# Rick0514/SimpleSLAM

Hardware: AMD Instinct MI355X
Metric: scans/s (65 k-pt scan vs 1 M-pt submap, LOAM 10 iters) + pose RMSE vs CPU ref (higher is better)
Workload: dtype f64; 1 GPU; pcr=loam, 65536-pt 64-beam scan vs 1000000-pt submap, 10 GN iters, early exit off, index rebuilt per call (previous call's bounding box and tile layout reused as checked hints), inputs in HBM; parallelism=single GPU, scans_cycled=8

## Files before the change

### simpleslam_amd/csrc/loam.hip

```cpp
#include <hip/hip_ext.h>

#include "pcr_internal.h"
#include "peer_exchange.h"
#include "small_math.h"

namespace pcr {



static constexpr int kNb = 8;
static constexpr uint32_t kNoPos = 0xffffffffu;
static constexpr uint32_t kKeyEmpty = 0xffffffffu;

struct Nb8 {
    double d[kNb];
    uint32_t idx[kNb];
    float x[kNb], y[kNb], z[kNb];
};

__device__ __forceinline__ bool knn_less(double d, uint32_t i, double d2, uint32_t i2) {
    return (d < d2) | ((d == d2) & (i < i2));
}

__device__ __forceinline__ double sqdist(double qx, double qy, double qz, float px, float py, float pz) {
// ... 121 lines not shown
            for (int t = 0; t < 9; ++t) {
                const uint2 r = sh.run[t][tid];
                const uint32_t len = r.y - r.x;
                const bool skip = (uint32_t)t == k && (uint32_t)t < n_runs && rem >= len;
                rem -= skip ? len : 0u; k += skip ? 1u : 0u;
            }
        }
        const uint2 r0 = sh.run[min(k, 9u)][tid];
        cur.k = k; cur.j = r0.x + rem; cur.e = r0.y; cur.nx = sh.run[min(k + 1u, 9u)][tid];
    }
    uint32_t nmax = n_mine;
#pragma unroll
    for (int m = 32; m >= 1; m >>= 1) nmax = max(nmax, (uint32_t)__shfl_xor((int)nmax, m, 64));
    const uint32_t groups = __builtin_amdgcn_readfirstlane((nmax + (uint32_t)kGroup - 1u) / (uint32_t)kGroup);
    float4 c[kGroup];
    if (groups) {
#pragma unroll
        for (int u = 0; u < kGroup; ++u) {
            const uint32_t pos = knn_cursor_step(cur, sh, tid);
            c[u] = pts[(uint32_t)u < n_mine ? pos : 0u];
        }
    }
    if (tl) { float t_ = 0.f; if (groups) { for (int u = 0; u < kGroup; ++u) t_ += c[u].x; } if (t_ == 1.2345e38f) key[0] = 0u; tl[9] = wall_clock64(); }
    for (uint32_t g = 0; g < groups; ++g) {
        float4 n[kGroup];
        if (g + 1u < groups) {
#pragma unroll
            for (int u = 0; u < kGroup; ++u) {
                const uint32_t pos = knn_cursor_step(cur, sh, tid);
                n[u] = pts[(g + 1u) * (uint32_t)kGroup + (uint32_t)u < n_mine ? pos : 0u];
            }
        } else {
#pragma unroll
            for (int u = 0; u < kGroup; ++u) n[u] = make_float4(0.f, 0.f, 0.f, 0.f);
        }
#pragma unroll
        for (int u = 0; u < kGroup; ++u) {
            const uint32_t seq = g * (uint32_t)kGroup + (uint32_t)u;
            const float dx = qxf - c[u].x, dy = qyf - c[u].y, dz = qzf - c[u].z;
            float d = dx * dx;
            d = __builtin_fmaf(dy, dy, d);
            d = __builtin_fmaf(dz, dz, d);
            uint32_t t = (__float_as_uint(d) & ~idmask) | (s0 + seq);
            t = (seq < n_mine && d <= gate_f) ? t : kKeyEmpty;
#pragma unroll
            for (int k = 0; k < kNb; ++k) { const uint32_t lo = min(key[k], t), hi = max(key[k], t); key[k] = lo; t = hi; }
            key[kNb] = min(key[kNb], t);
        }
#pragma unroll
        for (int u = 0; u < kGroup; ++u) c[u] = n[u];
    }
    if (tl) tl[10] = wall_clock64();
    return !inside ? 0 : (too_many ? 2 : 1);
}

__device__ __forceinline__ void knn_decode(const KnnRuns& sh, int tid, const uint32_t key[kNb + 1], uint32_t idmask, uint32_t pos[kNb]) {
    uint32_t P[9], off[9];
    uint32_t acc = 0;
#pragma unroll
    for (int t = 0; t < 9; ++t) { const uint2 r = sh.run[t][tid]; P[t] = acc; off[t] = r.x - acc; acc += r.y - r.x; }
#pragma unroll
    for (int j = 0; j < kNb; ++j) {
        const uint32_t seq = key[j] & idmask;
        uint32_t o = off[0];
#pragma unroll
        for (int t = 1; t < 9; ++t) o = seq >= P[t] ? off[t] : o;
        pos[j] = key[j] == kKeyEmpty ? kNoPos : seq + o;
    }
}

__device__ __forceinline__ double knn_list_bound(const uint32_t key[kNb + 1], uint32_t idmask) {
    if (key[kNb] == kKeyEmpty) return __longlong_as_double(0x7ff0000000000000ll);
    return (double)__uint_as_float(key[kNb] & ~idmask) * (1.0 - 1e-6);
}

struct NnCacheEntry {
    float4 nb[kNb];
    float q0[3];
    float l9;
    double x[3];
    uint32_t pidx[5];
    uint32_t flags;
};
static_assert(sizeof(NnCacheEntry) == 192, "cache entry layout");
static constexpr int kEntryVec = sizeof(NnCacheEntry) / 16;

__device__ __forceinline__ bool knn_from_cache(const NnCacheEntry& ce, double qx, double qy, double qz, Nb8& s, bool* moved) {
#pragma unroll
    for (int j = 0; j < kNb; ++j) {
        const float4 p = ce.nb[j];
        s.x[j] = p.x; s.y[j] = p.y; s.z[j] = p.z; s.idx[j] = __float_as_uint(p.w);
        const double d = sqdist(qx, qy, qz, p.x, p.y, p.z);
        s.d[j] = d == d ? d : __longlong_as_double(0x7ff0000000000000ll);
    }
    bool ord = true;
#pragma unroll
    for (int j = 0; j < 4; ++j) ord = ord & !knn_less(s.d[j + 1], s.idx[j + 1], s.d[j], s.idx[j]);
#pragma unroll
    for (int j = 5; j < kNb; ++j) ord = ord & !knn_less(s.d[j], s.idx[j], s.d[4], s.idx[4]);
    *moved = false;
    if (!__all(ord)) {
        uint32_t before[kNb];
#pragma unroll
        for (int j = 0; j < kNb; ++j) before[j] = s.idx[j];
        nb8_sort(s);
        bool mv = false;
#pragma unroll
        for (int j = 0; j < kNb; ++j) mv = mv | (before[j] != s.idx[j]);
        *moved = mv;
    }
    const double ex = qx - (double)ce.q0[0], ey = qy - (double)ce.q0[1], ez = qz - (double)ce.q0[2];
    const double delta = sqrt(ex * ex + ey * ey + ez * ez) * (1.0 + 1e-12) + 1e-13;
    const double slack = (double)ce.l9 - delta;
    return s.idx[4] != 0xffffffffu && slack > 0.0 && s.d[4] < slack * slack * (1.0 - 1e-12);
}

__device__ __forceinline__ void swap_d(double& a, double& b) { const double t = a; a = b; b = t; }

__device__ __forceinline__ void plane_qr_solve(double a[5][3], double x[3]) {
    double c[5] = {-1.0, -1.0, -1.0, -1.0, -1.0};
    int perm[3] = {0, 1, 2};
    double tau[3] = {0, 0, 0};
    double nu[3], nd[3];
    double maxn = 0;
#pragma unroll
    for (int j = 0; j < 3; ++j) {
        double s = 0;
#pragma unroll
        for (int i = 0; i < 5; ++i) s += a[i][j] * a[i][j];
        nd[j] = nu[j] = sqrt(s);
        if (nu[j] > maxn) maxn = nu[j];
    }
    const double eps = 2.220446049250313e-16;
    const double thr_helper = (maxn * eps) * (maxn * eps) / 5.0;
    const double downdate_thr = 1.4901161193847656e-08;
    int nonzero = 3;
#pragma unroll
    for (int k = 0; k < 3; ++k) {
        int big = k; double bign = nu[k];
#pragma unroll
        for (int j = k + 1; j < 3; ++j) if (nu[j] > bign) { bign = nu[j]; big = j; }
        const double big_sq = bign * bign;
        if (nonzero == 3 && big_sq < thr_helper * (double)(5 - k)) nonzero = k;
#pragma unroll
        for (int j = k + 1; j < 3; ++j) {
            if (big == j) {
#pragma unroll
                for (int i = 0; i < 5; ++i) swap_d(a[i][k], a[i][j]);
                swap_d(nu[k], nu[j]); swap_d(nd[k], nd[j]);
                const int t = perm[k]; perm[k] = perm[j]; perm[j] = t;
            }
        }
        double tail_sq = 0;
#pragma unroll
        for (int i = k + 1; i < 5; ++i) tail_sq += a[i][k] * a[i][k];
        const double c0 = a[k][k];
        const bool tiny = tail_sq <= 2.2250738585072014e-308;
        double beta_h = sqrt(c0 * c0 + tail_sq);
        beta_h = c0 >= 0 ? -beta_h : beta_h;
        const double den = c0 - beta_h;
#pragma unroll
        for (int i = k + 1; i < 5; ++i) { const double q = a[i][k] / den; a[i][k] = tiny ? 0.0 : q; }
        const double tau_h = (beta_h - c0) / beta_h;
        tau[k] = tiny ? 0.0 : tau_h;
        a[k][k] = tiny ? c0 : beta_h;
#pragma unroll
        for (int j = k + 1; j < 3; ++j) {
            double tmp = 0;
// ... 99 lines not shown
            in = d <= seed_sq;
            if (!in) out_min = fmin(out_min, d);
        }
        const unsigned long long m = __ballot(in);
        if (in) tab[n_in + (uint32_t)__popcll(m & ((1ull << lane) - 1ull))] = w;
        n_in += (uint32_t)__popcll(m);
    }
#pragma unroll
    for (int sft = 32; sft >= 1; sft >>= 1) out_min = fmin(out_min, __shfl_xor(out_min, sft, 64));
    __builtin_amdgcn_fence(__ATOMIC_RELEASE, "workgroup");
    for (uint32_t c = lane; c < n_in; c += 64) {
        const WaveCand me = tab[c];
        uint32_t rank = 0;
#pragma unroll 4
        for (uint32_t j = 0; j < n_in; ++j) {
            const WaveCand o = tab[j];
            rank += knn_less(o.d, o.idx, me.d, me.idx) ? 1u : 0u;
        }
        if (rank <= (uint32_t)kNb) { tab[kWaveTab + rank] = me; }
    }
    __builtin_amdgcn_fence(__ATOMIC_RELEASE, "workgroup");
#pragma unroll
    for (int j = 0; j < kNb; ++j) {
        if ((uint32_t)j < n_in) pos_out[j] = tab[kWaveTab + j].pos;
    }
    double nx = out_min;
    if (n_in > (uint32_t)kNb) nx = fmin(nx, tab[kWaveTab + kNb].d);
    *next_sq = fmin(max_sq, nx);
    return true;
}

static constexpr int kRowStride = 258;
static constexpr int kSparseMisses = 8;
struct MissExchange {
    uint32_t wcount[4];
    uint32_t fallback, pad_[3];
    uint32_t list[256];
    float qx[256], qy[256], qz[256];
    double seed[256];
    union alignas(16) {
        struct {
            uint32_t pos[kNb][256];
            double bound[256];
            uint32_t state[256];
            uint32_t keys[kNb + 1][256];
            uint32_t idmask[256];
        } res;
        double rows[8 * kRowStride];
    } u;
};
static_assert(offsetof(MissExchange, u) % 16 == 0 && (kRowStride * sizeof(double)) % 16 == 0 && sizeof(KnnRuns) % 16 == 0,
              "the chunk sums read two doubles of a row per instruction");

__device__ __forceinline__ uint32_t posted_owner(const MissExchange& ex, const uint32_t c[4], uint32_t m) {
    const uint32_t p1 = c[0], p2 = p1 + c[1], p3 = p2 + c[2];
    const uint32_t w = (m >= p1 ? 1u : 0u) + (m >= p2 ? 1u : 0u) + (m >= p3 ? 1u : 0u);
    const uint32_t first = w == 0u ? 0u : (w == 1u ? p1 : (w == 2u ? p2 : p3));
    return ex.list[w * 64u + (m - first)];
}

struct EntryWrite {
    uint32_t what;
    Nb8 s;
    float q[3];
    double bound_sq;
    double x[3];
    uint32_t flags;
};

__device__ __forceinline__ uint32_t entry_fields(const EntryWrite& w, float4 v[kEntryVec]) {
#pragma unroll
    for (int j = 0; j < kNb; ++j) v[j] = make_float4(w.s.x[j], w.s.y[j], w.s.z[j], __uint_as_float(w.s.idx[j]));
    v[kNb] = make_float4(w.q[0], w.q[1], w.q[2], __double2float_rd(sqrt(w.bound_sq) * (1.0 - 1e-15)));
    union { struct { double x[3]; uint32_t pidx[5]; uint32_t flags; } t; float4 v[3]; } tail;
    tail.t.x[0] = w.x[0]; tail.t.x[1] = w.x[1]; tail.t.x[2] = w.x[2];
#pragma unroll
    for (int j = 0; j < 5; ++j) tail.t.pidx[j] = w.s.idx[j];
    tail.t.flags = w.flags;
#pragma unroll
    for (int f = 0; f < 3; ++f) v[kNb + 1 + f] = tail.v[f];
    return ((w.what & 1u) ? 0x0ffu : 0u) | ((w.what & 2u) ? 0x100u : 0u) | ((w.what & 4u) ? 0xe00u : 0u);
}

static constexpr int kFewWriters = 8;
__device__ __forceinline__ void entry_store_lane(NnCacheEntry* __restrict__ mine_e, const EntryWrite& w) {
    if (w.what & 8u) mine_e->flags = 0;
    float4 v[kEntryVec];
    const uint32_t fields = entry_fields(w, v);
    float4* const dst = reinterpret_cast<float4*>(mine_e);
#pragma unroll
    for (int f = 0; f < kEntryVec; ++f) if ((fields >> f) & 1u) dst[f] = v[f];
}

__device__ __forceinline__ void entry_store_wave(NnCacheEntry* __restrict__ e0, const EntryWrite& w, float4* stage) {
    const int lane = threadIdx.x & 63;
    if (w.what & 8u) e0[lane].flags = 0;
    float4* const mine = stage + lane * kEntryVec;
    float4 mv[kEntryVec];
    const uint32_t fields = entry_fields(w, mv);
#pragma unroll
    for (int f = 0; f < kEntryVec; ++f) mine[f] = mv[f];
    __builtin_amdgcn_fence(__ATOMIC_RELEASE, "workgroup");
    float4* const dst = reinterpret_cast<float4*>(e0);
#pragma unroll
    for (int i = 0; i < kEntryVec; ++i) {
        const uint32_t c = (uint32_t)(i * 64 + lane);
        const uint32_t owner = c / (uint32_t)kEntryVec, f = c - owner * (uint32_t)kEntryVec;
        const uint32_t m = (uint32_t)__shfl((int)fields, (int)owner, 64);
        const float4 v = stage[c];
        if ((m >> f) & 1u) dst[c] = v;
    }
}

template <int kGroup>
__device__ __forceinline__ int loam_point(const LoamArgs& a, const GridHeader& h, const double* __restrict__ pose,
                                          float sx, float sy, float sz, bool valid, const NnCacheEntry& ce_in, bool have_entry,
                                          KnnRuns& sh, MissExchange& ex, double row[7], uint32_t nn_idx[5], uint32_t qi, int* how,
                                          bool* escaped, EntryWrite& ew, unsigned long long* tl, const bool all_search = false) {
    const double ox = (double)sx, oy = (double)sy, oz = (double)sz;
    const float px = (float)(pose[0] * ox + pose[4] * oy + pose[8] * oz + pose[12] * 1.0);
    const float py = (float)(pose[1] * ox + pose[5] * oy + pose[9] * oz + pose[13] * 1.0);
    const float pz = (float)(pose[2] * ox + pose[6] * oy + pose[10] * oz + pose[14] * 1.0);
    const double qx = (double)px, qy = (double)py, qz = (double)pz;
    const bool in_range = valid;
    bool active = valid && !h.empty && !h.overflow;
    if (a.use_tile) {
        const bool in_tile = qx >= a.tile_lo[0] && qx < a.tile_hi[0] && qy >= a.tile_lo[1] && qy < a.tile_hi[1] &&
                             qz >= a.tile_lo[2] && qz < a.tile_hi[2];
        if (!in_tile) { active = false; valid = false; }
    }
    *escaped = false;
    if (h.clamped && active) {
        const double fx = floor((qx - h.origin[0]) * h.inv_cell), fy = floor((qy - h.origin[1]) * h.inv_cell), fz = floor((qz - h.origin[2]) * h.inv_cell);
        const int cm = h.cut_mask;
        *escaped = ((cm & 1) && fx <= (double)kPad) || ((cm & 8) && fx >= (double)(h.dims[0] - kPad - 1)) ||
                   ((cm & 2) && fy <= (double)kPad) || ((cm & 16) && fy >= (double)(h.dims[1] - kPad - 1)) ||
                   ((cm & 4) && fz <= (double)kPad) || ((cm & 32) && fz >= (double)(h.dims[2] - kPad - 1));
    }
    Nb8 s;
    bool moved = false;
    const bool have_seed = have_entry && active && (ce_in.flags & 1u);
    bool hit = false;
    if (tl) { if (px + py + pz == 1.2345e38f) moved = true; tl[16] = wall_clock64(); }
    if (have_seed) hit = knn_from_cache(ce_in, qx, qy, qz, s, &moved);
    if (tl) { if (hit && s.d[4] == 1.2345e300) moved = true; tl[17] = wall_clock64(); }
    const int tid = threadIdx.x;
    const bool miss = active && !hit;
    KnnRanges own_ranges;
    own_ranges.inside = false;
#pragma unroll
    for (int r = 0; r < 9; ++r) { own_ranges.ra[r] = 0u; own_ranges.rb[r] = 0u; }
    if (__any(miss)) knn_ranges_issue(h, a.grid.cell_start, px, py, pz, miss, own_ranges);
    uint32_t posted[4] = {0u, 0u, 0u, 0u};
    if (!all_search) {
    const unsigned long long mb = __ballot(miss);
    if ((tid & 63) == 0) ex.wcount[tid >> 6] = (uint32_t)__popcll(mb);
    if (miss) {
        ex.list[(uint32_t)(tid & ~63) + __builtin_amdgcn_mbcnt_hi((uint32_t)(mb >> 32), __builtin_amdgcn_mbcnt_lo((uint32_t)mb, 0u))] = (uint32_t)tid;
        ex.qx[tid] = px; ex.qy[tid] = py; ex.qz[tid] = pz;
        double sb = a.c.knn_max_sq;
        if (have_seed) {
            double mx = s.d[0];
#pragma unroll
            for (int j = 1; j < kNb; ++j) mx = fmax(mx, s.d[j]);
            sb = fmin(sb, mx);
        }
        ex.seed[tid] = sb;
    }
    __syncthreads();
#pragma unroll
    for (int wv = 0; wv < 4; ++wv) posted[wv] = ex.wcount[wv];
    }
    if (tl) { if (posted[0] == 0x12345678u) moved = true; tl[2] = wall_clock64(); }
    bool self = false;
    uint32_t self_pos[kNb], self_state = 0u;
    double self_bound = 0.0;
    {
        const uint32_t n_miss = all_search ? 256u : posted[0] + posted[1] + posted[2] + posted[3];
        bool dense = n_miss > (uint32_t)kSparseMisses;
        if (n_miss && !dense) {
            if (tid == 0) ex.fallback = 0;
            __syncthreads();
            const int wave = tid >> 6;
            WaveCand* tab = reinterpret_cast<WaveCand*>(&sh) + (size_t)wave * (kWaveTab + 16);
            for (uint32_t m = wave; m < n_miss; m += 4) {
                const uint32_t owner = posted_owner(ex, posted, m);
                uint32_t rp[kNb];
                double nxt = 0.0;
                bool ins = false;
                const bool done = knn8_wave(h, a.grid.pts, a.grid.cell_start, (double)ex.qx[owner], (double)ex.qy[owner], (double)ex.qz[owner],
                                            a.c.knn_max_sq, ex.seed[owner], tab, rp, &nxt, &ins);
                if (!done) { if ((tid & 63) == 0) ex.fallback = 1; }
                else if ((tid & 63) == 0) {
#pragma unroll
// ... 117 lines not shown
    if (fit) {
        const double xn0 = sqrt(x[0] * x[0] + x[1] * x[1] + x[2] * x[2]);
        plane_ok = true;
#pragma unroll
        for (int i = 0; i < 5; ++i) {
            const double dot = x[0] * A[i][0] + x[1] * A[i][1] + x[2] * A[i][2];
            if (fabs(dot + 1.0) > a.c.plane_thresh * xn0) plane_ok = false;
        }
    }
    if (tl) { if (plane_ok && x[0] == 1.2345e300) x[1] = 0.0; tl[15] = wall_clock64(); }
    ew.what = 0u;
    if (a.nn_cache && in_range && !active) {
        ew.what = 8u;
    }
    if (a.nn_cache && active) ew.what = ((miss || moved) ? 1u : 0u) | (miss ? 2u : 0u) | ((miss || !reuse) ? 4u : 0u);
    ew.s = s;
    ew.q[0] = px; ew.q[1] = py; ew.q[2] = pz;
    ew.bound_sq = bound_sq;
    ew.x[0] = x[0]; ew.x[1] = x[1]; ew.x[2] = x[2];
    ew.flags = (searched ? 1u : 0u) | (real5 ? 2u : 0u) | (plane_ok ? 4u : 0u);
    if (tl) tl[4] = wall_clock64();
    if (!valid) return 4;
    if (!searched) return 1;
#pragma unroll
    for (int j = 0; j < 5; ++j) nn_idx[j] = s.idx[j];
    if (!gate_knn) return 1;
    if (!plane_ok) return 2;
    const double xn = sqrt(x[0] * x[0] + x[1] * x[1] + x[2] * x[2]);
    const double dist = (qx * x[0] + qy * x[1] + qz * x[2] + 1.0) / xn;
    const float r2 = sx * sx + sy * sy + sz * sz;
    const float rr = sqrtf(sqrtf(r2));
    const double w = 1 - 0.9 * fabs(dist) / (double)rr;
    if (!(w > a.c.point_thresh)) return 3;
    const double n0 = x[0] / xn, n1 = x[1] / xn, n2 = x[2] / xn;
    const double s0 = w * n0, s1 = w * n1, s2 = w * n2;
    row[0] = s0; row[1] = s1; row[2] = s2;
    row[3] = s1 * (-qz) + s2 * qy;
    row[4] = s0 * qz + s2 * (-qx);
    row[5] = s0 * (-qy) + s1 * qx;
    row[6] = w * dist;
    return 0;
}

static constexpr double kBigStep = 0.12;
struct Prologue {
    double pose[16];
    int done;
    int big_step;
};

__device__ __forceinline__ void lds_dma16(const float4* src, float4* lds_wave_base) {
    const uint32_t base = __builtin_amdgcn_readfirstlane((uint32_t)(uintptr_t)(__attribute__((address_space(3))) void*)lds_wave_base);
    asm volatile("s_mov_b32 m0, %1\n\ts_nop 0\n\tglobal_load_lds_dwordx4 %0, off" ::"v"(src), "s"(base) : "m0", "memory");
}

struct LoamHead {
    const double* partials;
    LoamState* state;
    const double* reduced;
    uint32_t n_partials;
};

__device__ __forceinline__ double readlane_f64(double v, int lane) {
    return __hiloint2double(__builtin_amdgcn_readlane(__double2hiint(v), lane), __builtin_amdgcn_readlane(__double2loint(v), lane));
}

struct HeadLoads { int prev_done; double prev_pose_t, red; double pv[32]; };
__device__ __forceinline__ void loam_head_issue(const LoamHead hd, int k, HeadLoads& L) {
    const int t = threadIdx.x, comp = t & 31, slice = t >> 5;
    const LoamState* prev = &hd.state[(k + 1) & 1];
    L.prev_done = prev->done;
    L.prev_pose_t = prev->pose[t & 15];
    const double* const part0 = hd.partials + (size_t)((k + 1) & 1) * kMaxPartials * kAccum + comp;
    const uint32_t last = hd.n_partials ? hd.n_partials - 1u : 0u;
#pragma unroll
    for (int u = 0; u < 32; ++u) {
        const uint32_t b = (uint32_t)slice + 8u * u;
        L.pv[u] = part0[(size_t)(b < last ? b : last) * kAccum];
    }
    L.red = *(hd.reduced ? hd.reduced + comp : part0);
}

__device__ bool loam_prologue(const LoamHead hd, const HeadLoads& L, const LoamArgs& a, int k, double* sh_sum , Prologue* sh,
                              unsigned long long* tl = nullptr, const float4* pre_src = nullptr, float4* pre_dst = nullptr) {
    const LoamState* prev = &hd.state[(k + 1) & 1];
    LoamState* cur = &hd.state[k & 1];
    const int t = threadIdx.x;
    if (k == 0) {
        if (t < 16) sh->pose[t] = a.init_pose[t];
        if (t == 0) { sh->done = 0; sh->big_step = 0; }
        if (blockIdx.x == 0 && t == 0) {
            for (int i = 0; i < 16; ++i) cur->pose[i] = a.init_pose[i];
            cur->done = 0; cur->converged = 0; cur->iters_run = 0; cur->fail = 0;
        }
        __syncthreads();
        return false;
    }
    const int comp = t & 31, slice = t >> 5;
    const uint32_t n_rows = hd.n_partials;
    const int prev_done = L.prev_done;
    const double prev_pose_t = L.prev_pose_t;
    const double* const part0 = hd.partials + (size_t)((k + 1) & 1) * kMaxPartials * kAccum + comp;
    const double red = L.red;
    double acc = 0.0;
#pragma unroll
    for (int u = 0; u < 32; ++u) acc += ((uint32_t)slice + 8u * u < n_rows) ? L.pv[u] : 0.0;
    for (uint32_t b0 = (uint32_t)slice + 256u; b0 < n_rows; b0 += 128u) {
        const uint32_t last = n_rows - 1u;
        double w[16];
#pragma unroll
        for (int u = 0; u < 16; ++u) { const uint32_t b = b0 + 8u * u; w[u] = part0[(size_t)(b < last ? b : last) * kAccum]; }
#pragma unroll
        for (int u = 0; u < 16; ++u) acc += (b0 + 8u * u < n_rows) ? w[u] : 0.0;
    }
    if (hd.reduced) acc = slice == 0 ? red : 0.0;
    sh_sum[slice * 32 + comp] = acc;
    if (t < 16) sh->pose[t] = prev_pose_t;
    __syncthreads();
    if (tl) tl[7] = wall_clock64();
    if (pre_dst) {
        const float4* src = pre_src ? pre_src : reinterpret_cast<const float4*>(hd.partials) + (size_t)t * kEntryVec;
#pragma unroll
        for (int f = 0; f < kEntryVec; ++f) lds_dma16(src + f, pre_dst + f * 256);
    }
    if (prev_done) {
        if (t == 0) sh->done = 1;
        if (blockIdx.x == 0 && t == 0) { *cur = *prev; __hip_atomic_store(&a.result->progress, (k << 1) | 1, __ATOMIC_RELAXED, __HIP_MEMORY_SCOPE_SYSTEM); }
        __syncthreads();
        return true;
    }
    if (t < 32) {
        double v = sh_sum[t];
#pragma unroll
        for (int s = 1; s < 8; ++s) v += sh_sum[s * 32 + t];
        sh_sum[t] = v;
    }
    __syncthreads();
    double* const sh_x = sh_sum + 112;
    if (t < 64) {
        const int i = t >> 3, j = t & 7;
        const bool in = i < 6 && j < 7;
        double v = 0.0;
        if (in) {
            const int r = i < j ? i : j, c = i < j ? j : i;
            v = j < 6 ? sh_sum[r * 6 - (r * (r - 1)) / 2 + (c - r)] : -sh_sum[21 + i];
        }
        const double maxd = fmax(fmax(fmax(fabs(sh_sum[0]), fabs(sh_sum[6])), fmax(fabs(sh_sum[11]), fabs(sh_sum[15]))),
                                 fmax(fabs(sh_sum[18]), fabs(sh_sum[20])));
        bool weak = false;
#pragma unroll
        for (int kk = 0; kk < 6; ++kk) {
            const double pk = readlane_f64(v, kk * 9);
            const double aik = __shfl(v, (t & ~7) | kk, 64), akj = __shfl(v, kk * 8 + j, 64);
            weak = weak || !(fabs(pk) > 1e-6 * maxd);
            const double rp = 1.0 / pk;
            if (in) v = (i == kk) ? akj * rp : v - (aik * rp) * akj;
        }
        if (in && j == 6) sh_x[i] = v;
        if (t == 0) sh_x[6] = weak ? 1.0 : 0.0;
    }
    __syncthreads();
    if (tl) tl[11] = wall_clock64();
    if (t < 64) {
        double x[6];
#pragma unroll
        for (int r = 0; r < 6; ++r) x[r] = sh_x[r];
        const bool weak = sh_x[6] != 0.0;
        const int oc = (t >> 2) & 3, orow = t & 3;
        double pcol[4];
#pragma unroll
        for (int kk = 0; kk < 4; ++kk) pcol[kk] = sh->pose[oc * 4 + kk];
        const bool writer = blockIdx.x == 0 && t == 0;
        if (weak || a.trace) {
            double JtJ[36], rhs[6];
            int q = 0;
            for (int r = 0; r < 6; ++r) for (int c = r; c < 6; ++c) { JtJ[r * 6 + c] = JtJ[c * 6 + r] = sh_sum[q++]; }
            for (int r = 0; r < 6; ++r) rhs[r] = -sh_sum[21 + r];
            if (weak) ldlt6_solve(JtJ, rhs, x);
            if (writer && a.trace) {
                LoamTrace* tr = &a.trace[k - 1];
                for (int i = 0; i < 36; ++i) tr->JtJ[i] = JtJ[i];
                for (int i = 0; i < 6; ++i) tr->JtE[i] = -rhs[i];
                tr->n = (int64_t)sh_sum[27];
                tr->cache_hits = (int64_t)sh_sum[28]; tr->searches = (int64_t)sh_sum[29];
            }
        }
        const double n = sh_sum[27];
        int done = 0, conv = 0, fail = 0, big = 0;
        bool step = false;
        double np = 0.0, nr = 0.0;
        if (hd.reduced && sh_sum[kSlotRankFail] != 0.0) { done = 1; fail = 2; }
        else if (sh_sum[kSlotEscapes] != 0.0) { done = 1; fail = 3; }
        else if (n < 6.0) { done = 1; fail = 1; }
        else {
            np = sqrt(x[0] * x[0] + x[1] * x[1] + x[2] * x[2]);
            nr = sqrt(x[3] * x[3] + x[4] * x[4] + x[5] * x[5]);
            if (a.c.early_exit && np <= a.c.pos_conv && nr <= a.c.rot_conv) { done = 1; conv = 1; }
            else step = true;
        }
        if (fail) { for (int r = 0; r < 6; ++r) x[r] = 0.0; }
        if (k >= a.c.iters) done = 1;
        double mine = prev_pose_t;
        if (step) {
            double E[16];
            se3_exp(x, E);
            double* const sh_E = sh_sum + 128;
            if (t == 0) {
#pragma unroll
                for (int i = 0; i < 16; ++i) sh_E[i] = E[i];
            }
            __builtin_amdgcn_fence(__ATOMIC_RELEASE, "workgroup");
            __builtin_amdgcn_wave_barrier();
            double s = 0;
#pragma unroll
            for (int kk = 0; kk < 4; ++kk) s += sh_E[kk * 4 + orow] * pcol[kk];
            mine = s;
            big = (!done && np + 10.0 * nr > kBigStep) ? 1 : 0;
        }
        if (step && t < 16) sh->pose[t] = mine;
        if (t == 0) { sh->done = done; sh->big_step = big; }
        if (blockIdx.x == 0) {
            if (t < 16) cur->pose[t] = mine;
            if (t == 0) {
                cur->done = done; cur->converged = conv; cur->fail = fail; cur->iters_run = k;
                __hip_atomic_store(&a.result->progress, (k << 1) | (done ? 1 : 0), __ATOMIC_RELAXED, __HIP_MEMORY_SCOPE_SYSTEM);
                if (a.trace) { for (int i = 0; i < 6; ++i) a.trace[k - 1].x[i] = x[i]; }
            }
        }
    }
    __syncthreads();
    return sh->done != 0;
}

template <int kGroup, int kWavesPerSimd>
__global__ __launch_bounds__(256, kWavesPerSimd) void loam_iterate_kernel(double* const partials, LoamState* const state, const double* const reduced,
                                                                          const uint32_t n_partials, const int k, NnCacheEntry* const nn_cache,
                                                                          const float* const src, const LoamArgs a) {
    const unsigned long long t_entry = wall_clock64();
    const LoamHead hd = {partials, state, reduced, n_partials};
    HeadLoads head;
    loam_head_issue(hd, k, head);
    __shared__ double sh_sum[8 * 32];
    __shared__ Prologue sh_pro;
    struct SearchLds { KnnRuns knn; MissExchange ex; };
    constexpr size_t kStage = (size_t)kEntryVec * 256 * sizeof(float4);
    __shared__ __attribute__((aligned(16))) unsigned char sh_ov[sizeof(SearchLds) > kStage ? sizeof(SearchLds) : kStage];
    KnnRuns& sh_knn = reinterpret_cast<SearchLds*>(sh_ov)->knn;
    MissExchange& sh_ex = reinterpret_cast<SearchLds*>(sh_ov)->ex;
    double* const sh_rows = sh_ex.u.rows;
    const int tid = threadIdx.x;
    unsigned long long* const tl = (a.timeline && tid == 0) ? a.timeline + ((size_t)k * kMaxPartials + blockIdx.x) * kTimelineSlots : nullptr;
    if (tl) tl[0] = t_entry;
    uint32_t blk = blockIdx.x;
    if ((gridDim.x & 7u) == 0) blk = (blockIdx.x & 7u) * (gridDim.x >> 3) + (blockIdx.x >> 3);
    float4* const sh_pre = reinterpret_cast<float4*>(sh_ov);
    GridHeader h;
    {
        static_assert(sizeof(GridHeader) % 4 == 0, "header copied by words");
        const __attribute__((address_space(4))) uint32_t* const hw = (const __attribute__((address_space(4))) uint32_t*)(uintptr_t)a.grid.hdr;
        uint32_t* const w = reinterpret_cast<uint32_t*>(&h);
#pragma unroll
        for (size_t i = 0; i < sizeof(GridHeader) / 4; ++i) w[i] = hw[i];
    }
    float pre_x = 0.f, pre_y = 0.f, pre_z = 0.f;
    const bool use_cache = k > 0 && nn_cache != nullptr;
    const float4* pre_src = nullptr;
    const uint32_t qpb = 256u;
    {
        const uint32_t q = blk * qpb + (uint32_t)tid;
        const float* sp = a.n_src ? src + (size_t)(q < a.n_src ? q : a.n_src - 1u) * a.src_stride
                                  : reinterpret_cast<const float*>(partials);
        pre_x = sp[0]; pre_y = sp[1]; pre_z = sp[2];
        pre_src = (use_cache && q < a.n_src) ? reinterpret_cast<const float4*>(nn_cache + q) : nullptr;
    }
    if (loam_prologue(hd, head, a, k, sh_sum, &sh_pro, tl, pre_src, use_cache ? sh_pre + (tid & ~63) : nullptr)) {
        asm volatile("s_waitcnt vmcnt(0)" ::: "memory");
        return;
    }
    if (tl) tl[1] = wall_clock64();
    double pose[16];
#pragma unroll
    for (int i = 0; i < 16; ++i) pose[i] = sh_pro.pose[i];

    const int e = tid & 31, ch = tid >> 5;
    int er = 7, ec = 7;
    {
        int q = 0;
#pragma unroll
        for (int r = 0; r < 6; ++r) {
#pragma unroll
            for (int c = r; c < 6; ++c) { if (q == e) { er = r; ec = c; } ++q; }
        }
        if (e >= 21 && e < 27) { er = e - 21; ec = 6; }
    }
    double acc = 0.0;
    uint32_t n_hit = 0, n_search = 0, n_esc = 0;
    for (uint32_t base = blk * qpb; base < a.n_src; base += gridDim.x * qpb) {
        const uint32_t q = base + tid;
        const bool valid = q < a.n_src;
        double row[7] = {0, 0, 0, 0, 0, 0, 0};
        uint32_t nn[5] = {0xffffffffu, 0xffffffffu, 0xffffffffu, 0xffffffffu, 0xffffffffu};
        int how = 0;
        bool esc = false;
        EntryWrite ew;
        float sx = pre_x, sy = pre_y, sz = pre_z;
        union { NnCacheEntry e; float4 v[kEntryVec]; } ce;
        ce.e.flags = 0;
        bool all_search = false;
        if (base == blk * qpb) {
            all_search = sh_pro.big_step != 0;
            if (use_cache) asm volatile("s_waitcnt vmcnt(0)" ::: "memory");
            if (use_cache && valid && !sh_pro.big_step) {
#pragma unroll
                for (int f = 0; f < kEntryVec; ++f) ce.v[f] = sh_pre[f * 256 + tid];
            }
            __syncthreads();
        } else {
            sx = sy = sz = 0.f;
            if (valid) {
                const float* sp = src + (size_t)q * a.src_stride;
                sx = sp[0]; sy = sp[1]; sz = sp[2];
                if (use_cache) ce.e = nn_cache[q];
            }
        }
        const int st = loam_point<kGroup>(a, h, pose, sx, sy, sz, valid, ce.e, use_cache && valid && !all_search, sh_knn, sh_ex, row, nn, q, &how, &esc, ew,
                                          base == blk * qpb ? tl : nullptr, all_search);
        if (valid && (a.dbg_status || a.dbg_nn || a.dbg_rows)) {
            const size_t oi = (size_t)q;
            if (a.dbg_status) a.dbg_status[oi] = (int8_t)st;
            if (a.dbg_nn) { for (int j = 0; j < 5; ++j) a.dbg_nn[oi * 5 + j] = (int32_t)nn[j]; }
            if (a.dbg_rows) { for (int j = 0; j < 7; ++j) a.dbg_rows[oi * 7 + j] = st == 0 ? row[j] : 0.0; }
        }
#pragma unroll
        for (int c = 0; c < 7; ++c) sh_rows[c * kRowStride + tid] = st == 0 ? row[c] : 0.0;
        sh_rows[7 * kRowStride + tid] = st == 0 ? 1.0 : 0.0;
        __syncthreads();
        if (tl && base == blk * qpb) tl[18] = wall_clock64();
        n_hit += (uint32_t)__popcll(__ballot(how == 1)); n_search += (uint32_t)__popcll(__ballot(how == 2));
        if (h.clamped) n_esc += (uint32_t)__popcll(__ballot(esc));
        if (e < 28) {
            const double2* ra = reinterpret_cast<const double2*>(sh_rows + er * kRowStride + ch * 32);
            const double2* rb = reinterpret_cast<const double2*>(sh_rows + ec * kRowStride + ch * 32);
#pragma unroll 8
            for (int i = 0; i < 16; ++i) {
                const double2 va = ra[i], vb = rb[i];
                acc += va.x * vb.x;
                acc += va.y * vb.y;
            }
        }
        if (tl && base == blk * qpb) { if (acc == 1.2345e300) n_hit = 0u; tl[19] = wall_clock64(); }
        __syncthreads();
        const int writers = __popcll(__ballot(ew.what != 0u));
        if (writers) {
            if (writers > kFewWriters) entry_store_wave(nn_cache + (q - (uint32_t)(tid & 63)), ew, reinterpret_cast<float4*>(sh_ov) + (tid >> 6) * (64 * kEntryVec));
            else entry_store_lane(nn_cache + q, ew);
        }
        if (base + gridDim.x * qpb < a.n_src) __syncthreads();
    }
    if (tl) tl[5] = wall_clock64();
    sh_sum[ch * 32 + e] = e < 28 ? acc : 0.0;
    __shared__ uint32_t sh_cnt[12];
    if ((tid & 63) == 0) { sh_cnt[(tid >> 6) * 2] = n_hit; sh_cnt[(tid >> 6) * 2 + 1] = n_search; sh_cnt[8 + (tid >> 6)] = n_esc; }
    __syncthreads();
    if (tid < 32) {
        double v = sh_sum[tid];
#pragma unroll
        for (int c = 1; c < 8; ++c) v += sh_sum[c * 32 + tid];
        if (tid == 28) v = (double)(sh_cnt[0] + sh_cnt[2] + sh_cnt[4] + sh_cnt[6]);
        if (tid == 29) v = (double)(sh_cnt[1] + sh_cnt[3] + sh_cnt[5] + sh_cnt[7]);
        if (tid == kSlotEscapes) v = (double)(sh_cnt[8] + sh_cnt[9] + sh_cnt[10] + sh_cnt[11]);
        partials[((size_t)(k & 1) * kMaxPartials + blockIdx.x) * kAccum + tid] = v;
    }
    if (tl) tl[6] = wall_clock64();
}

__global__ __launch_bounds__(256) void loam_finalize_kernel(const double* const partials, LoamState* const state, const double* const reduced,
                                                            const uint32_t n_partials, const int k, const LoamArgs a) {
    __shared__ double sh_sum[8 * 32];
    __shared__ Prologue sh_pro;
    const LoamHead hd = {partials, state, reduced, n_partials};
    HeadLoads head;
    loam_head_issue(hd, k, head);
    loam_prologue(hd, head, a, k, sh_sum, &sh_pro);
    if (threadIdx.x == 0) {
        double T[16];
        for (int i = 0; i < 16; ++i) T[i] = sh_pro.pose[i];
        t2se3(T);
        const LoamState* cur = &state[k & 1];
        LoamResult* r = a.result;
        for (int i = 0; i < 16; ++i) r->pose[i] = T[i];
        r->converged = cur->converged; r->iters_run = cur->iters_run; r->fail = cur->fail;
        r->grid_overflow = a.grid.hdr->overflow; r->grid_empty = a.grid.hdr->empty; r->grid_cells = a.grid.hdr->n_cells;
        r->grid_stale = a.grid.hdr->stale;
        __threadfence_system();
        __hip_atomic_store(&r->pad, 1, __ATOMIC_RELEASE, __HIP_MEMORY_SCOPE_SYSTEM);
    }
}

__device__ __forceinline__ double loam_fold_own_rows(const LoamArgs& a, int k, int comp, int slice) {
    const int done = a.state[k & 1].done;
    const double* const part0 = a.partials + (size_t)(k & 1) * kMaxPartials * kAccum + comp;
    const uint32_t last = a.n_partials ? a.n_partials - 1u : 0u;
    double pv[32];
#pragma unroll
    for (int u = 0; u < 32; ++u) { const uint32_t b = (uint32_t)slice + 8u * u; pv[u] = part0[(size_t)(b < last ? b : last) * kAccum]; }
    double acc = 0.0;
#pragma unroll
    for (int u = 0; u < 32; ++u) acc += ((uint32_t)slice + 8u * u < a.n_partials) ? pv[u] : 0.0;
    for (uint32_t b = (uint32_t)slice + 256u; b < a.n_partials; b += 8u) acc += part0[(size_t)b * kAccum];
    return done ? 0.0 : acc;
}

__global__ __launch_bounds__(256) void loam_reduce_kernel(const LoamArgs a, const int k, double* __restrict__ out) {
    __shared__ double sh_sum[8 * 32];
    const int t = threadIdx.x, comp = t & 31, slice = t >> 5;
    const double acc = loam_fold_own_rows(a, k, comp, slice);
    sh_sum[slice * 32 + comp] = acc;
    __syncthreads();
    if (t < 32) {
        double v = sh_sum[t];
#pragma unroll
        for (int s = 1; s < 8; ++s) v += sh_sum[s * 32 + t];
        if (t == kSlotRankFail) v = (a.rank_fail || a.grid.hdr->overflow) ? 1.0 : 0.0;
        out[t] = v;
    }
}

__global__ __launch_bounds__(256) void loam_peer_exchange_kernel(const LoamArgs a, const int k, const PeerComm pc, const double seq, double* __restrict__ out) {
    __shared__ double sh_sum[8 * 32];
    const int t = threadIdx.x, comp = t & 31, slice = t >> 5;
    const double acc = loam_fold_own_rows(a, k, comp, slice);
    sh_sum[slice * 32 + comp] = acc;
    __syncthreads();
    double v = 0.0;
    if (t < 32) {
        v = sh_sum[t];
#pragma unroll
        for (int s = 1; s < 8; ++s) v += sh_sum[s * 32 + t];
        if (t == kSlotRankFail) v = (a.rank_fail || a.grid.hdr->overflow) ? 1.0 : 0.0;
// ... 46 lines not shown
```

### simpleslam_amd/csrc/loam_host.hip

```cpp

#include <algorithm>

#include "handle.h"

using namespace pcr;
using namespace pcr::host;

namespace {

double grid_cell_for(double max_sq) {
    double r = sqrt(max_sq > 0 ? max_sq : 1.0), c = 1.0;
    while (c < r) c *= 2.0;
    while (c * 0.5 >= r) c *= 0.5;
    return c;
}

int ensure_loam_buffers(pcr_handle* h) {
    H_TRY(h->loam.state.reserve(2 * sizeof(LoamState)));
    H_TRY(h->loam.partials.reserve((size_t)2 * kMaxPartials * kAccum * sizeof(double)));
    H_TRY(h->loam.reduced.reserve(kAccum * sizeof(double)));
    const int iters = std::max(1, h->prm.loam_iters);
    if (h->prm.record_trace) H_TRY(h->loam.trace.reserve((size_t)iters * sizeof(LoamTrace)));
    H_TRY(h->loam.result.ensure());
    if (h->comm.host_ar) H_TRY(h->loam.red.ensure(kAccum));
    return 0;
}

void fill_loam_args(pcr_handle* h, LoamArgs* a, const float* d_src, size_t n_src, size_t stride_floats, const double pose[16]) {
    memset(a, 0, sizeof(*a));
    a->src = d_src; a->n_src = (uint32_t)n_src; a->src_stride = (uint32_t)stride_floats;
    a->grid = h->grid.view();
    a->c.knn_max_sq = h->prm.loam_knn_max_sq; a->c.plane_thresh = h->prm.loam_plane_thresh;
    a->c.point_thresh = h->prm.loam_point_thresh; a->c.pos_conv = h->prm.loam_pos_conv; a->c.rot_conv = h->prm.loam_rot_conv;
    a->c.iters = h->prm.loam_iters; a->c.early_exit = h->prm.loam_early_exit;
    memcpy(a->init_pose, pose, 16 * sizeof(double));
    a->state = h->loam.state.as<LoamState>();
    a->partials = h->loam.partials.as<double>();
    a->reduced = nullptr;
    a->n_partials = loam_grid_blocks((uint32_t)n_src);
    h->loam.last_blocks = a->n_partials;
    a->trace = h->prm.record_trace ? h->loam.trace.as<LoamTrace>() : nullptr;
    a->result = h->loam.result.dev;
    a->coresident = h->prm.loam_coresident == 1;
    if (h->prm.loam_disable_cache == 0 && h->loam.nn_cache.reserve((n_src + 1) * 192) == hipSuccess) a->nn_cache = (NnCacheEntry*)h->loam.nn_cache.p;
    if (h->prm.record_timeline == 1 && h->loam.timeline.reserve((size_t)(std::max(1, h->prm.loam_iters) + 1) * kMaxPartials * kTimelineSlots * sizeof(unsigned long long)) == hipSuccess)
        a->timeline = h->loam.timeline.as<unsigned long long>();
    a->use_tile = h->use_tile;
    for (int d = 0; d < 3; ++d) { a->tile_lo[d] = h->tile_lo[d]; a->tile_hi[d] = h->tile_hi[d]; }
}

}

namespace pcr {
namespace host {

int build_target(pcr_handle* h, const float* d_dst, size_t n_dst, size_t stride_floats) {
    double cell = 1.0;
    if (h->method == kLoam) cell = grid_cell_for(h->prm.loam_knn_max_sq);
    h->grid.no_hints = h->prm.index_no_hints != 0;
    hipError_t e = h->grid.build(d_dst, n_dst, stride_floats, cell, h->stream, &h->err, 0.0, 0, h->clamp.use ? &h->clamp : nullptr, h->method == kLoam);
    if (e != hipSuccess) return 1;
    h->tgt_ptr = d_dst; h->tgt_n = n_dst; h->tgt_stride = stride_floats; h->have_target = true;
    return 0;
}
int rebuild_stale_target(pcr_handle* h) {
    h->grid.hint_margin = 8; h->grid.cells_hint = 0;
    return build_target(h, h->tgt_ptr, h->tgt_n, h->tgt_stride);
}


int set_clamp_from_scan(pcr_handle* h, const float* d_src, size_t n_src, size_t stride_floats, const double pose[16]) {
    if (!n_src) return fail(h, "target bounding box too large for the dense index and the scan is empty");
    if (h->src_grid.build(d_src, n_src, stride_floats, 1.0, h->stream, &h->err) != hipSuccess) return 1;
    GridHeader sh;
    H_TRY(hipMemcpyAsync(&sh, h->src_grid.header.p, sizeof sh, hipMemcpyDeviceToHost, h->stream));
    H_TRY(hipStreamSynchronize(h->stream));
    if (sh.empty) return fail(h, "target bounding box too large for the dense index and the scan has no finite point");
    double lo[3], hi[3], mlo[3] = {1e300, 1e300, 1e300}, mhi[3] = {-1e300, -1e300, -1e300};
    for (int d = 0; d < 3; ++d) { lo[d] = sh.origin[d]; hi[d] = sh.origin[d] + sh.dims[d] * sh.cell; }
    for (int c = 0; c < 8; ++c) {
        const double p[3] = {c & 1 ? hi[0] : lo[0], c & 2 ? hi[1] : lo[1], c & 4 ? hi[2] : lo[2]};
        for (int r = 0; r < 3; ++r) {
            const double v = pose[r] * p[0] + pose[4 + r] * p[1] + pose[8 + r] * p[2] + pose[12 + r];
            mlo[r] = std::min(mlo[r], v); mhi[r] = std::max(mhi[r], v);
        }
    }
    for (int d = 0; d < 3; ++d) {
        if (!(mlo[d] == mlo[d] && mhi[d] == mhi[d])) return fail(h, "target bounding box too large for the dense index and the initial pose is not finite");
        h->clamp.lo[d] = mlo[d] - h->clamp_margin; h->clamp.hi[d] = mhi[d] + h->clamp_margin;
    }
    h->clamp.use = 1;
    return 0;
}

int set_clamp_from_target_sample(pcr_handle* h) {
    const size_t n = h->tgt_n, stride_b = h->tgt_stride * 4;
    if (!n || !h->tgt_ptr) return fail(h, "target bounding box too large for the dense index");
    const size_t step = std::max<size_t>(1, n / 4096), m = (n + step - 1) / step;
    std::vector<float> xyz(m * 3);
    H_TRY(hipMemcpy2DAsync(xyz.data(), 12, h->tgt_ptr, stride_b * step, 12, m, hipMemcpyDeviceToHost, h->stream));
    H_TRY(hipStreamSynchronize(h->stream));
    for (int d = 0; d < 3; ++d) {
        std::vector<double> v;
        v.reserve(m);
        for (size_t i = 0; i < m; ++i) { const float a = xyz[i * 3], b = xyz[i * 3 + 1], c = xyz[i * 3 + 2]; if (std::isfinite(a) && std::isfinite(b) && std::isfinite(c)) v.push_back((double)xyz[i * 3 + d]); }
        if (v.empty()) return fail(h, "target bounding box too large for the dense index and no finite point in its sample");
        std::sort(v.begin(), v.end());
        const double q_lo = v[(size_t)(0.02 * (double)(v.size() - 1))], q_hi = v[(size_t)(0.98 * (double)(v.size() - 1) + 0.5)];
        const double pad = 0.5 * (q_hi - q_lo) + 20.0;
        h->clamp.lo[d] = q_lo - pad; h->clamp.hi[d] = q_hi + pad;
    }
    h->clamp.use = 1;
    return 0;
}

}
}

namespace {

int check_grid_overflow(pcr_handle* h, int overflow, uint64_t need_cells, const float* d_src = nullptr, size_t n_src = 0, size_t stride_floats = 0,
                        const double* pose = nullptr) {
    if (!overflow) return 0;
    if (need_cells > 4000000000ull && h->method == kLoam && d_src && pose && !h->clamp.use) {
        if (set_clamp_from_scan(h, d_src, n_src, stride_floats, pose)) return 1;
        if (build_target(h, h->tgt_ptr, h->tgt_n, h->tgt_stride)) return 1;
        return 2;
// ... 263 lines not shown
```

### simpleslam_amd/csrc/pcr_internal.h

```cpp
#pragma once
#include <hip/hip_runtime.h>
#include <hip/hip_ext.h>
#include <stdint.h>
#include <functional>
#include <string>
#include <vector>

#include <stdlib.h>

#include "../../include/pcr_hip.h"
#include "grid_plan.h"

namespace pcr {

struct GridHeader {
    double origin[3];
    double org[3];
    double cell;
    double inv_cell;
    int32_t dims[3];
    uint32_t n_points;
    uint64_t n_cells;
    int32_t overflow;
    int32_t empty;
    double shift;
    int32_t pcl_mode;
    float inv_leaf_f;
    int32_t min_b[3];
    int32_t too_fine;
    float sum_sq;
    int32_t clamped;
    int32_t cut_mask;
    unsigned long long sum_sq_u;
    int32_t stale;
    int32_t pad2_;
};
__host__ __device__ inline double grid_sum_sq(const GridHeader& h) { return h.sum_sq_u ? (double)h.sum_sq_u : (double)h.sum_sq; }

struct ClampBox { double lo[3], hi[3]; int32_t use, pad_; };

struct HeaderTwin { GridHeader* hdr; GridHeader* mirror; uint64_t capacity; double cell; };

struct GridView {
    const GridHeader* hdr;
    const float4* pts;
    const uint32_t* cell_start;
};

static constexpr int kPad = 2;
static constexpr double kProgressWindow = 1048576.0;

struct Pose16 { double m[16]; };

struct LoamState {
    double pose[16];
    int32_t done;
    int32_t converged;
    int32_t iters_run;
    int32_t fail;
};

static constexpr int kAccum = 32;
static constexpr int kSlotRankFail = 30;
static constexpr int kSlotEscapes = 31;
static constexpr int kMaxPartials = 512;
static constexpr int kTimelineSlots = 24;

struct LoamConsts {
    double knn_max_sq, plane_thresh, point_thresh, pos_conv, rot_conv;
    int32_t iters, early_exit;
};

struct LoamResult {
    double pose[16];
    int32_t converged, iters_run, fail, grid_overflow, grid_empty, pad;
    uint64_t grid_cells;
    int32_t grid_stale;
    int32_t progress;
};

struct LoamTrace {
    double JtJ[36];
    double JtE[6];
    double x[6];
    int64_t n;
    int64_t cache_hits, searches;
};

struct NnCacheEntry;

struct LoamArgs {
    const float* src;
    uint32_t n_src;
    uint32_t src_stride;
    GridView grid;
    LoamConsts c;
    double init_pose[16];
    LoamState* state;
    double* partials;
    const double* reduced;
    uint32_t n_partials;
    LoamTrace* trace;
    LoamResult* result;
    int8_t* dbg_status;
    double* dbg_rows;
    int32_t* dbg_nn;
    struct NnCacheEntry* nn_cache;
    int32_t use_tile;
    double tile_lo[3], tile_hi[3];
    int32_t coresident;
    int32_t rank_fail;
    unsigned long long* timeline;
};

struct DeviceBuf {
    void* p = nullptr;
    size_t cap = 0;
    DeviceBuf() = default;
    DeviceBuf(const DeviceBuf&) = delete;
    DeviceBuf& operator=(const DeviceBuf&) = delete;
    ~DeviceBuf() { release(); }
    hipError_t reserve(size_t bytes);
    void release();
    template <class T> T* as() const { return static_cast<T*>(p); }
};

static constexpr uint32_t kNdtUnprepared = 0xffffffffu;
struct TileTail {
    uint32_t* vox_slot; uint32_t* list; uint32_t* count; uint32_t* count_next;
    int32_t min_points; uint32_t capacity;
    const uint8_t* mask; int32_t mshift;
};
struct BuildFilter {
    std::function<hipError_t()> enqueue_mask;
    const uint8_t* mask = nullptr;
    int mshift = 0;
    bool applied = false;
    bool want_tail = false;
    TileTail tail = {};
    bool tail_applied = false;
};

struct GridIndex : BuildHints {
    DeviceBuf sorted, cell_count, cell_start, block_sums, bbox_partials, header, keys, ranks, ticket;
    DeviceBuf kept;
    DeviceBuf tiled, bin_count, bin_start, tile_sq;
    DeviceBuf layout[2];
    GridHeader* header_mirror = nullptr;
    GridIndex* twin = nullptr;
    double twin_cell = 0.0;
    hipError_t ensure_tables(hipStream_t s, std::string* err);
    void confirm() { hint_ok = valid && tiled_shift >= 0; }
    size_t n_points = 0;
    size_t reserve_points = 0;
    bool valid = false;
    GridView view() const {
        return GridView{header.as<GridHeader>(), sorted.as<float4>(), cell_start.as<uint32_t>()};
    }
    hipError_t build(const float* d_pts, size_t n, size_t stride_floats, double cell, hipStream_t s,
                     std::string* err, double shift = 0.0, int pcl_mode = 0, const ClampBox* clamp = nullptr, bool allow_hint = false,
                     BuildFilter* filter = nullptr);
    hipError_t enqueue_build(BuildPlan& p, BuildRequest& rq, size_t n_res, const ClampBox& cb, hipStream_t s, std::string* err, BuildFilter* filter);
    hipError_t grow_cells(uint64_t need_cells, std::string* err);
    hipError_t enqueue_density(hipStream_t s);
    void release();
};

struct VgicpVoxel {
    double mean[3];
    double cov[6];
    double w;
    uint32_t n, pad;
};

struct RoiView {
    const GridHeader* lat;
    const uint8_t* mask;
    uint32_t* escapes;
    int32_t mshift;
    int32_t filtered;
    uint32_t* count;
};
__host__ __device__ inline uint32_t roi_macro(const GridHeader& h, int mshift, int cx, int cy, int cz) {
    const uint32_t m0 = ((uint32_t)h.dims[0] + (1u << mshift) - 1u) >> mshift, m1 = ((uint32_t)h.dims[1] + (1u << mshift) - 1u) >> mshift;
    return (((uint32_t)cz >> mshift) * m1 + ((uint32_t)cy >> mshift)) * m0 + ((uint32_t)cx >> mshift);
}
__host__ __device__ inline bool roi_mask_holds_cell(const GridHeader& h, const uint8_t* mask, int mshift, uint32_t key) {
    const uint32_t d0 = (uint32_t)h.dims[0], d1 = (uint32_t)h.dims[1], row = key / d0, cz = row / d1;
    return mask[roi_macro(h, mshift, (int)(key - row * d0), (int)(row - cz * d1), (int)cz)] != 0;
}
// ... 198 lines not shown
```

Measured before the change: 4202 scans/s.

## Store NN cache as tiled field-major SoA and hoist cache prefetch wait

Changes the per-query nearest-neighbour cache from an array of 192-byte structs to a tiled layout where each 64-query tile stores each 16-byte field contiguously. Cache loads and stores become coalesced per field across a wave, which replaces the LDS-staged wave store path and the lane-wise path with a single strided store. The prologue's trailing barrier is merged with the cache-prefetch wait so the prefetched entry is read into registers before one shared barrier. This costs a different buffer size calculation and some scattered partial-field writes, and it adds new timeline probes.

Measured after the change: 4338 scans/s, median of 6. +3.2%, better.

```diff
diff --git a/simpleslam_amd/csrc/loam.hip b/simpleslam_amd/csrc/loam.hip
--- a/simpleslam_amd/csrc/loam.hip
+++ b/simpleslam_amd/csrc/loam.hip
@@ -227,8 +227,12 @@
     uint32_t pidx[5];
     uint32_t flags;
 };
-static_assert(sizeof(NnCacheEntry) == 192, "cache entry layout");
-static constexpr int kEntryVec = sizeof(NnCacheEntry) / 16;
+static constexpr int kEntryVec = kCacheFields;
+static_assert(sizeof(NnCacheEntry) == kEntryVec * sizeof(float4), "cache entry fields");
+static constexpr int kEntryStride = 64;
+__device__ __forceinline__ float4* entry_field(float4* cache, uint32_t q) {
+    return cache + (size_t)(q >> 6) * (kEntryVec * 64) + (q & 63u);
+}
 
 __device__ __forceinline__ bool knn_from_cache(const NnCacheEntry& ce, double qx, double qy, double qz, Nb8& s, bool* moved) {
 #pragma unroll
@@ -494,34 +498,12 @@
     return ((w.what & 1u) ? 0x0ffu : 0u) | ((w.what & 2u) ? 0x100u : 0u) | ((w.what & 4u) ? 0xe00u : 0u);
 }
 
-static constexpr int kFewWriters = 8;
-__device__ __forceinline__ void entry_store_lane(NnCacheEntry* __restrict__ mine_e, const EntryWrite& w) {
-    if (w.what & 8u) mine_e->flags = 0;
+__device__ __forceinline__ void entry_store(float4* __restrict__ mine, const EntryWrite& w) {
+    if (w.what & 8u) reinterpret_cast<uint32_t*>(mine + (kEntryVec - 1) * kEntryStride)[3] = 0;
     float4 v[kEntryVec];
     const uint32_t fields = entry_fields(w, v);
-    float4* const dst = reinterpret_cast<float4*>(mine_e);
-#pragma unroll
-    for (int f = 0; f < kEntryVec; ++f) if ((fields >> f) & 1u) dst[f] = v[f];
-}
-
-__device__ __forceinline__ void entry_store_wave(NnCacheEntry* __restrict__ e0, const EntryWrite& w, float4* stage) {
-    const int lane = threadIdx.x & 63;
-    if (w.what & 8u) e0[lane].flags = 0;
-    float4* const mine = stage + lane * kEntryVec;
-    float4 mv[kEntryVec];
-    const uint32_t fields = entry_fields(w, mv);
-#pragma unroll
-    for (int f = 0; f < kEntryVec; ++f) mine[f] = mv[f];
-    __builtin_amdgcn_fence(__ATOMIC_RELEASE, "workgroup");
-    float4* const dst = reinterpret_cast<float4*>(e0);
-#pragma unroll
-    for (int i = 0; i < kEntryVec; ++i) {
-        const uint32_t c = (uint32_t)(i * 64 + lane);
-        const uint32_t owner = c / (uint32_t)kEntryVec, f = c - owner * (uint32_t)kEntryVec;
-        const uint32_t m = (uint32_t)__shfl((int)fields, (int)owner, 64);
-        const float4 v = stage[c];
-        if ((m >> f) & 1u) dst[c] = v;
-    }
+#pragma unroll
+    for (int f = 0; f < kEntryVec; ++f) if ((fields >> f) & 1u) mine[f * kEntryStride] = v[f];
 }
 
 template <int kGroup>
@@ -805,7 +787,8 @@
 }
 
 __device__ bool loam_prologue(const LoamHead hd, const HeadLoads& L, const LoamArgs& a, int k, double* sh_sum , Prologue* sh,
-                              unsigned long long* tl = nullptr, const float4* pre_src = nullptr, float4* pre_dst = nullptr) {
+                              unsigned long long* tl = nullptr, const float4* pre_src = nullptr, float4* pre_dst = nullptr,
+                              const bool caller_closes = false) {
     const LoamState* prev = &hd.state[(k + 1) & 1];
     LoamState* cur = &hd.state[k & 1];
     const int t = threadIdx.x;
@@ -816,7 +799,7 @@
             for (int i = 0; i < 16; ++i) cur->pose[i] = a.init_pose[i];
             cur->done = 0; cur->converged = 0; cur->iters_run = 0; cur->fail = 0;
         }
-        __syncthreads();
+        if (!caller_closes) __syncthreads();
         return false;
     }
     const int comp = t & 31, slice = t >> 5;
@@ -842,9 +825,8 @@
     __syncthreads();
     if (tl) tl[7] = wall_clock64();
     if (pre_dst) {
-        const float4* src = pre_src ? pre_src : reinterpret_cast<const float4*>(hd.partials) + (size_t)t * kEntryVec;
-#pragma unroll
-        for (int f = 0; f < kEntryVec; ++f) lds_dma16(src + f, pre_dst + f * 256);
+#pragma unroll
+        for (int f = 0; f < kEntryVec; ++f) lds_dma16(pre_src + f * kEntryStride, pre_dst + f * 256);
     }
     if (prev_done) {
         if (t == 0) sh->done = 1;
@@ -951,13 +933,14 @@
             }
         }
     }
+    if (caller_closes) return false;
     __syncthreads();
     return sh->done != 0;
 }
 
 template <int kGroup, int kWavesPerSimd>
 __global__ __launch_bounds__(256, kWavesPerSimd) void loam_iterate_kernel(double* const partials, LoamState* const state, const double* const reduced,
-                                                                          const uint32_t n_partials, const int k, NnCacheEntry* const nn_cache,
+                                                                          const uint32_t n_partials, const int k, float4* const nn_cache,
                                                                           const float* const src, const LoamArgs a) {
     const unsigned long long t_entry = wall_clock64();
     const LoamHead hd = {partials, state, reduced, n_partials};
@@ -994,16 +977,34 @@
         const float* sp = a.n_src ? src + (size_t)(q < a.n_src ? q : a.n_src - 1u) * a.src_stride
                                   : reinterpret_cast<const float*>(partials);
         pre_x = sp[0]; pre_y = sp[1]; pre_z = sp[2];
-        pre_src = (use_cache && q < a.n_src) ? reinterpret_cast<const float4*>(nn_cache + q) : nullptr;
-    }
-    if (loam_prologue(hd, head, a, k, sh_sum, &sh_pro, tl, pre_src, use_cache ? sh_pre + (tid & ~63) : nullptr)) {
+        const uint32_t tiles = (a.n_src + 63u) >> 6;
+        if (use_cache) pre_src = entry_field(nn_cache, ((q >> 6) < tiles ? (q & ~63u) : (tiles << 6)) + (q & 63u));
+    }
+    union EntryRegs { NnCacheEntry e; float4 v[kEntryVec]; };
+    if (loam_prologue(hd, head, a, k, sh_sum, &sh_pro, tl, pre_src, use_cache ? sh_pre + (tid & ~63) : nullptr, true)) {
         asm volatile("s_waitcnt vmcnt(0)" ::: "memory");
         return;
     }
+    EntryRegs ce0;
+    ce0.e.flags = 0;
+    if (use_cache) {
+        asm volatile("s_waitcnt vmcnt(0)" ::: "memory");
+        if (tl) tl[21] = wall_clock64();
+        if (blk * qpb + (uint32_t)tid < a.n_src) {
+#pragma unroll
+            for (int f = 0; f < kEntryVec; ++f) ce0.v[f] = sh_pre[f * 256 + tid];
+            if (tl) { float t_ = 0.f; for (int f = 0; f < kEntryVec; ++f) t_ += ce0.v[f].x; if (t_ == 1.2345e38f) ce0.e.flags = 0u; }
+        }
+        if (tl) tl[22] = wall_clock64();
+    }
+    __syncthreads();
+    if (tl) tl[23] = wall_clock64();
+    if (sh_pro.done) return;
     if (tl) tl[1] = wall_clock64();
     double pose[16];
 #pragma unroll
     for (int i = 0; i < 16; ++i) pose[i] = sh_pro.pose[i];
+    if (tl) { double t_ = 0.0; for (int i = 0; i < 16; ++i) t_ += pose[i]; if (t_ == 1.2345e300) pose[12] = 0.0; tl[20] = wall_clock64(); }
 
     const int e = tid & 31, ch = tid >> 5;
     int er = 7, ec = 7;
@@ -1027,23 +1028,22 @@
         bool esc = false;
         EntryWrite ew;
         float sx = pre_x, sy = pre_y, sz = pre_z;
-        union { NnCacheEntry e; float4 v[kEntryVec]; } ce;
+        EntryRegs ce;
         ce.e.flags = 0;
         bool all_search = false;
         if (base == blk * qpb) {
             all_search = sh_pro.big_step != 0;
-            if (use_cache) asm volatile("s_waitcnt vmcnt(0)" ::: "memory");
-            if (use_cache && valid && !sh_pro.big_step) {
-#pragma unroll
-                for (int f = 0; f < kEntryVec; ++f) ce.v[f] = sh_pre[f * 256 + tid];
-            }
-            __syncthreads();
+            ce = ce0;
         } else {
             sx = sy = sz = 0.f;
             if (valid) {
                 const float* sp = src + (size_t)q * a.src_stride;
                 sx = sp[0]; sy = sp[1]; sz = sp[2];
-                if (use_cache) ce.e = nn_cache[q];
+                if (use_cache) {
+                    const float4* const mine = entry_field(nn_cache, q);
+#pragma unroll
+                    for (int f = 0; f < kEntryVec; ++f) ce.v[f] = mine[f * kEntryStride];
+                }
             }
         }
         const int st = loam_point<kGroup>(a, h, pose, sx, sy, sz, valid, ce.e, use_cache && valid && !all_search, sh_knn, sh_ex, row, nn, q, &how, &esc, ew,
@@ -1072,12 +1072,7 @@
             }
         }
         if (tl && base == blk * qpb) { if (acc == 1.2345e300) n_hit = 0u; tl[19] = wall_clock64(); }
-        __syncthreads();
-        const int writers = __popcll(__ballot(ew.what != 0u));
-        if (writers) {
-            if (writers > kFewWriters) entry_store_wave(nn_cache + (q - (uint32_t)(tid & 63)), ew, reinterpret_cast<float4*>(sh_ov) + (tid >> 6) * (64 * kEntryVec));
-            else entry_store_lane(nn_cache + q, ew);
-        }
+        if (__ballot(ew.what != 0u)) entry_store(entry_field(nn_cache, q), ew);
         if (base + gridDim.x * qpb < a.n_src) __syncthreads();
     }
     if (tl) tl[5] = wall_clock64();
diff --git a/simpleslam_amd/csrc/loam_host.hip b/simpleslam_amd/csrc/loam_host.hip
--- a/simpleslam_amd/csrc/loam_host.hip
+++ b/simpleslam_amd/csrc/loam_host.hip
@@ -42,7 +42,7 @@
     a->trace = h->prm.record_trace ? h->loam.trace.as<LoamTrace>() : nullptr;
     a->result = h->loam.result.dev;
     a->coresident = h->prm.loam_coresident == 1;
-    if (h->prm.loam_disable_cache == 0 && h->loam.nn_cache.reserve((n_src + 1) * 192) == hipSuccess) a->nn_cache = (NnCacheEntry*)h->loam.nn_cache.p;
+    if (h->prm.loam_disable_cache == 0 && h->loam.nn_cache.reserve(loam_cache_bytes(n_src)) == hipSuccess) a->nn_cache = h->loam.nn_cache.as<float4>();
     if (h->prm.record_timeline == 1 && h->loam.timeline.reserve((size_t)(std::max(1, h->prm.loam_iters) + 1) * kMaxPartials * kTimelineSlots * sizeof(unsigned long long)) == hipSuccess)
         a->timeline = h->loam.timeline.as<unsigned long long>();
     a->use_tile = h->use_tile;
diff --git a/simpleslam_amd/csrc/pcr_internal.h b/simpleslam_amd/csrc/pcr_internal.h
--- a/simpleslam_amd/csrc/pcr_internal.h
+++ b/simpleslam_amd/csrc/pcr_internal.h
@@ -87,7 +87,9 @@
     int64_t cache_hits, searches;
 };
 
-struct NnCacheEntry;
+static constexpr int kCacheFields = 12;
+static constexpr size_t kCacheTileBytes = (size_t)kCacheFields * 64 * 16;
+static inline size_t loam_cache_bytes(size_t n_src) { return ((n_src + 63) / 64 + 1) * kCacheTileBytes; }
 
 struct LoamArgs {
     const float* src;
@@ -105,7 +107,7 @@
     int8_t* dbg_status;
     double* dbg_rows;
     int32_t* dbg_nn;
-    struct NnCacheEntry* nn_cache;
+    float4* nn_cache;
     int32_t use_tile;
     double tile_lo[3], tile_hi[3];
     int32_t coresident;
```
